# rapidsai/cudf

Hardware: NVIDIA H100
Metric: sort_by_key_rows_per_s (higher is better)
Workload: dtype int64

## Files before the change

cudf_b200/csrc/radix_sort.cu:

```cuda
#include "common.cuh"
#include "device_utils.cuh"

#include <algorithm>
#include <cmath>
#include <cstdlib>
#include <type_traits>

namespace b2 {
namespace {

constexpr int RADIX_BITS = 8;
constexpr int RADIX      = 256;
constexpr uint32_t FLAG_AGG  = 1u << 30;
constexpr uint32_t FLAG_INCL = 2u << 30;
constexpr uint32_t VAL_MASK  = (1u << 30) - 1;

struct pass_plan {
  int32_t trivial;
  int32_t key_src;
  int32_t key_dst;
  int32_t idx_src;
  int32_t idx_dst;
  int32_t last;
  int32_t hybrid;
// ... 784 lines not shown
    }
    if constexpr (RANGE) {
      dstd[j] = (uint8_t)d;
      if (q < tile_n) static_cast<UK*>(s_kdst[d])[dst[j]] = untwiddle_rt<UK>(k, a.kind, desc);
    } else if (write_keys && q < tile_n && (!(MIX || EST) || dst[j] != 0xFFFFFFFFu)) {
      if (!a.pairs && pl.last && !pl.hybrid) k = untwiddle_rt<UK>(k, a.kind, desc);
      kdst[dst[j]] = k;
    }
  }
  if (a.pairs) {
    ranker_barrier(THREADS);
#pragma unroll
    for (int i = 0; i < IPT; ++i) s_vals[pos[i]] = idx[i];
    ranker_barrier(THREADS);
    VT* idst = reinterpret_cast<VT*>(pl.idx_dst == 0 ? a.idx_bufs[0] : (pl.idx_dst == 1 ? a.idx_bufs[1] : a.idx_bufs[2]));
#pragma unroll
    for (int j = 0; j < IPT; ++j) {
      const uint32_t q = j * THREADS + tid;
      if constexpr (RANGE) {
        if (q < tile_n) static_cast<VT*>(s_vdst[dstd[j]])[dst[j]] = s_vals[q];
      } else {
        if (q < tile_n && (!(MIX || EST) || dst[j] != 0xFFFFFFFFu)) idst[dst[j]] = s_vals[q];
      }
    }
  }
}

template <typename UK, bool MIX = false>
__global__ void finalize_kernel(pass_args a, int64_t n, int raw, int pre_idx_buf, int carry_bytes)
{
  if (a.ctl->any_pass != 0) return;
  if (carry_bytes) {
    const int64_t stride = (int64_t)gridDim.x * blockDim.x;
    for (int64_t i = (int64_t)blockIdx.x * blockDim.x + threadIdx.x; i < n; i += stride) {
      if (carry_bytes == 8) reinterpret_cast<uint64_t*>(a.idx_bufs[0])[i] = static_cast<const uint64_t*>(a.val_in)[i];
      else reinterpret_cast<uint32_t*>(a.idx_bufs[0])[i] = static_cast<const uint32_t*>(a.val_in)[i];
      if (a.keep_keys && raw) {
        UK k = static_cast<const UK*>(a.key_bufs[0])[i];
        if constexpr (MIX) k = (UK)mix64((uint64_t)k);
        static_cast<UK*>(const_cast<void*>(a.key_bufs[1]))[i] = k;
      }
    }
    return;
  }
  const int64_t stride = (int64_t)gridDim.x * blockDim.x;
  for (int64_t i = (int64_t)blockIdx.x * blockDim.x + threadIdx.x; i < n; i += stride) {
    if (a.pairs) {
      if (raw) a.idx_bufs[0][i] = (int32_t)i;
      else if (pre_idx_buf != 0) a.idx_bufs[0][i] = a.idx_bufs[1][i];
      if (a.keep_keys && raw) {
        UK k = static_cast<const UK*>(a.key_bufs[0])[i];
        if constexpr (MIX) k = (UK)mix64((uint64_t)k);
        static_cast<UK*>(const_cast<void*>(a.key_bufs[1]))[i] = k;
      }
    } else {
      static_cast<UK*>(const_cast<void*>(a.key_bufs[1]))[i] = static_cast<const UK*>(a.key_bufs[0])[i];
    }
  }
}

constexpr int FIX_THREADS = 256;
constexpr int FIX_IPT     = 8;
constexpr int FIX_TILE    = FIX_THREADS * FIX_IPT;
constexpr int FIX_HALO    = 64;

struct seg_walk {
  int left, before;
  bool all_equal, cut;
};
template <typename UK, int FIX_FAST, typename KeyAt>
__device__ __forceinline__ seg_walk segment_walk(const KeyAt& key_at, UK k, int shift, int lmax, int rmax)
{
  const UK pf = k >> shift;
  seg_walk w{0, 0, true, false};
  bool in_l = true, in_r = true;
#pragma unroll
  for (int s = 1; s <= FIX_FAST; ++s) {
    const UK ol = key_at(-s);
    const UK orr = key_at(s);
    in_l = in_l && s <= lmax && (UK)(ol >> shift) == pf;
    in_r = in_r && s <= rmax && (UK)(orr >> shift) == pf;
    w.left += in_l ? 1 : 0;
    w.before += (in_l && ol <= k) ? 1 : 0;
    w.before += (in_r && orr < k) ? 1 : 0;
    w.all_equal = w.all_equal && (!in_l || ol == k) && (!in_r || orr == k);
  }
  int right = 0;
  if (in_l) {
    for (;;) {
      if (w.left == lmax) { w.cut = lmax == FIX_HALO; break; }
      const UK o = key_at(-w.left - 1);
      if ((UK)(o >> shift) != pf) break;
      ++w.left;
      w.before += o <= k ? 1 : 0;
      w.all_equal = w.all_equal && o == k;
    }
  }
  if (in_r) {
    right = FIX_FAST;
    for (;;) {
      if (right == rmax) { w.cut = w.cut || rmax == FIX_HALO; break; }
      const UK o = key_at(right + 1);
      if ((UK)(o >> shift) != pf) break;
      ++right;
      w.before += o < k ? 1 : 0;
      w.all_equal = w.all_equal && o == k;
    }
  }
  return w;
}

template <typename UK, typename VT, int FIX_FAST>
__global__ void __launch_bounds__(FIX_THREADS) segment_fix_kernel(pass_args a, int64_t n)
{
  if (!a.ctl->hybrid || a.ctl->fix_fast != (FIX_FAST ? 1 : 0)) return;
  __shared__ UK sk[FIX_TILE + 2 * FIX_HALO];
  const int shift = a.ctl->fix_shift;
  const UK* __restrict__ keys = static_cast<const UK*>(a.ctl->fix_key_buf == 1 ? a.key_bufs[1] : a.key_bufs[2]);
  const VT* __restrict__ vin  = reinterpret_cast<const VT*>(a.ctl->fix_idx_buf == 1 ? a.idx_bufs[1] : a.idx_bufs[2]);
  VT* __restrict__ vout = reinterpret_cast<VT*>(a.idx_bufs[0]);
  UK* __restrict__ kout = static_cast<UK*>(const_cast<void*>(a.key_bufs[1]));
  const UK desc = (UK)a.desc_mask;
  const int64_t ntiles = (n + FIX_TILE - 1) / FIX_TILE;
  for (int64_t tile = blockIdx.x; tile < ntiles; tile += gridDim.x) {
    const int64_t base = tile * FIX_TILE;
    __syncthreads();
    for (int q = threadIdx.x; q < FIX_TILE + 2 * FIX_HALO; q += FIX_THREADS) {
      const int64_t g = base - FIX_HALO + q;
      sk[q] = (g >= 0 && g < n) ? ld_stream(keys + g) : UK(0);
    }
    __syncthreads();
#pragma unroll
    for (int j = 0; j < FIX_IPT; ++j) {
      const int i = j * FIX_THREADS + threadIdx.x;
      const int64_t gi = base + i;
      if (gi >= n) continue;
      VT v{};
      if (a.pairs) v = ld_stream(vin + gi);
      const UK k  = sk[FIX_HALO + i];
      const int lmax = (int)(gi < FIX_HALO ? gi : (int64_t)FIX_HALO);
      const int rmax = (int)(n - 1 - gi < FIX_HALO ? n - 1 - gi : (int64_t)FIX_HALO);
      const seg_walk w = segment_walk<UK, FIX_FAST>([&](int o) { return sk[FIX_HALO + i + o]; }, k, shift, lmax, rmax);
      int64_t dst = gi - w.left + w.before;
      if (w.cut) {
        dst = gi;
        if (!w.all_equal) atomicOr(&a.ctl->overflow, 1u);
      }
      if (a.pairs) vout[dst] = v;
      else kout[dst] = untwiddle_rt<UK>(k, a.kind, desc);
    }
  }
}

constexpr int RANGE_THREADS     = 512;
constexpr int RANGE_WARPS       = RANGE_THREADS / 32;
constexpr int RANGE_IPT         = RANGE_CAP / RANGE_THREADS;
constexpr int RANGE_BUCKET_BITS = 13;
constexpr int RANGE_BUCKETS     = 1 << RANGE_BUCKET_BITS;
constexpr int RANGE_BUCKET_CAP  = FIX_HALO;
constexpr int RANGE_SLOTS       = RANGE_BUCKETS + RANGE_BUCKETS / 16;

size_t range_sort_smem(bool est)
{
  return 128 + sizeof(uint64_t) * (RANGE_CAP + 2) +
         (est ? sizeof(uint32_t) * (RANGE_SLOTS + RANGE_CAP) : sizeof(uint32_t) * RANGE_BUCKETS + sizeof(uint16_t) * RANGE_CAP);
}

__global__ void range_bounds_kernel(pass_args a, int64_t n, uint32_t* __restrict__ bounds, int nranges)
{
  const int i = blockIdx.x * blockDim.x + threadIdx.x;
  if (i > nranges) return;
  const uint64_t* __restrict__ keys = static_cast<const uint64_t*>(a.ctl->fix_key_buf == 1 ? a.key_bufs[1] : a.key_bufs[2]);
  const int sh = a.ctl->range_shift;
  const uint64_t mask = (uint64_t)nranges - 1;
  int64_t lo = 0, hi = n;
  while (lo < hi) {
    const int64_t mid = (lo + hi) >> 1;
    if ((int64_t)((keys[mid] >> sh) & mask) < i) lo = mid + 1;
    else hi = mid;
  }
  bounds[i] = (uint32_t)lo;
}

struct range_window {
  int base;
  bool bulk;
};
template <typename T>
__device__ __forceinline__ range_window range_window_load(T* sdst, const T* __restrict__ g, int64_t s, int m, uint32_t mbar)
{
  constexpr int PER = 16 / sizeof(T);
  const int off  = (int)((reinterpret_cast<uintptr_t>(g) & 15) / sizeof(T));
  const bool bulk = (reinterpret_cast<uintptr_t>(g) % sizeof(T)) == 0 && s >= off && m + off >= PER;
  const int bulk_rows = bulk ? (m + off) / PER * PER : 0;
  if (bulk) {
    if constexpr (EMU_BUILD) {
      for (int q = threadIdx.x; q < bulk_rows; q += RANGE_THREADS) sdst[q] = g[q - off];
    } else {
      if (threadIdx.x == 0) bulk_copy_to_smem(sdst, g - off, (uint32_t)(sizeof(T) * bulk_rows), mbar);
    }
    for (int r = bulk_rows - off + (int)threadIdx.x; r < m; r += RANGE_THREADS) sdst[off + r] = g[r];
  } else {
    for (int q = threadIdx.x; q < m; q += RANGE_THREADS) sdst[q] = ld_stream(g + q);
  }
  return {bulk ? off : 0, bulk};
}

__global__ void __launch_bounds__(RADIX) range_est_bounds_kernel(pass_args a, uint32_t cap, uint32_t* __restrict__ est)
{
  __shared__ uint32_t s_lb[RADIX + 1];
  __shared__ uint32_t s_wsum[RADIX / 32];
  constexpr int R = RADIX * RADIX;
  const int d7 = blockIdx.x, d6 = threadIdx.x;
  const uint64_t* __restrict__ keys = static_cast<const uint64_t*>(a.ctl->fix_key_buf == 1 ? a.key_bufs[1] : a.key_bufs[2]);
  auto count = [&](int e) { return min(a.ctl->base[1][7][e] - (uint32_t)e * cap, cap); };
  const uint32_t before = warp_sum(d6 < d7 ? count(d6) : 0u);
  if ((d6 & 31) == 0) s_wsum[d6 >> 5] = before;
  const uint32_t w0 = (uint32_t)d7 * cap, wn = count(d7);
  uint32_t lo = 0, hi = wn;
  while (lo < hi) {
    const uint32_t mid = (lo + hi) >> 1;
    if ((int)((keys[w0 + mid] >> 48) & 255u) < d6) lo = mid + 1;
    else hi = mid;
  }
  s_lb[d6] = lo;
  if (d6 == 0) s_lb[RADIX] = wn;
  __syncthreads();
  uint32_t dense = 0;
  for (int w = 0; w < RADIX / 32; ++w) dense += s_wsum[w];
  const uint32_t end = s_lb[d6 + 1];
  const int i = d7 * RADIX + d6;
  est[i]         = w0 + lo;
  est[R + i]     = end > lo ? end - lo : 0u;
  est[2 * R + i] = dense + lo;
}

#ifdef B2_RANGE_PROBE
constexpr int RANGE_PROBE_CTAS   = 1 << 17;
constexpr int RANGE_PROBE_STAMPS = 8;
__device__ long long g_range_probe[RANGE_PROBE_STAMPS + 2][RANGE_PROBE_CTAS];
void* g_range_probe_ptr()
{
  void* p = nullptr;
  cudaGetSymbolAddress(&p, g_range_probe);
  return p;
}
#define RANGE_PROBE_STAMP(i)                                                                  \
  do {                                                                                        \
    if (threadIdx.x == 0 && blockIdx.x < RANGE_PROBE_CTAS) g_range_probe[i][blockIdx.x] = clock64(); \
  } while (0)
#define RANGE_PROBE_SYNC() __syncthreads()
#else
#define RANGE_PROBE_STAMP(i) do {} while (0)
#define RANGE_PROBE_SYNC() do {} while (0)
#endif

__device__ __attribute__((noinline)) uint32_t range_rank_keys(const uint32_t* s_ord, const uint64_t* sk, uint32_t start, uint32_t end,
                                                              uint32_t r, uint64_t k)
{
  uint32_t before = 0;
  for (uint32_t q = start; q < end; ++q) {
    const uint32_t rq = s_ord[q] & 0xffffu;
    const uint64_t kq = sk[rq];
    before += (kq < k || (kq == k && rq < r)) ? 1u : 0u;
  }
  return before;
}

template <typename VT, bool EST = false>
__global__ void __launch_bounds__(RANGE_THREADS, 1) range_sort_kernel(pass_args a, const uint32_t* __restrict__ bounds)
{
  RANGE_PROBE_STAMP(0);
  using UK = uint64_t;
  B2_DYNAMIC_SMEM(smem_raw);
  uint32_t* s_misc = reinterpret_cast<uint32_t*>(smem_raw);
  UK* s_keys       = reinterpret_cast<UK*>(smem_raw + 128);
  VT* s_vals       = reinterpret_cast<VT*>(s_keys);
  uint32_t* s_cnt  = reinterpret_cast<uint32_t*>(s_keys + RANGE_CAP + 2);
  uint16_t* s_perm = reinterpret_cast<uint16_t*>(s_cnt + (EST ? RANGE_SLOTS : RANGE_BUCKETS));
  uint32_t* s_ord  = reinterpret_cast<uint32_t*>(s_perm);

  const int tid = threadIdx.x, lane = tid & 31, warp = tid >> 5;
  const int64_t s = bounds[blockIdx.x];
  int m;
  int64_t o = s;
  if constexpr (EST) {
    m = (int)bounds[gridDim.x + blockIdx.x];
    o = bounds[2 * gridDim.x + blockIdx.x];
  } else {
    m = (int)(bounds[blockIdx.x + 1] - s);
  }
  if (m == 0) return;
  if (m > RANGE_CAP) {
    if (tid == 0) atomicOr(&a.ctl->overflow, 1u);
    return;
  }
#ifdef B2_RANGE_PROBE
  if (tid == 0 && blockIdx.x < RANGE_PROBE_CTAS) {
    unsigned smid;
    asm volatile("mov.u32 %0, %%smid;" : "=r"(smid));
    g_range_probe[RANGE_PROBE_STAMPS][blockIdx.x]     = smid;
    g_range_probe[RANGE_PROBE_STAMPS + 1][blockIdx.x] = m;
  }
#endif
  const UK* __restrict__ keys = static_cast<const UK*>(a.ctl->fix_key_buf == 1 ? a.key_bufs[1] : a.key_bufs[2]) + s;
  const VT* __restrict__ vin  = reinterpret_cast<const VT*>(a.ctl->fix_idx_buf == 1 ? a.idx_bufs[1] : a.idx_bufs[2]) + s;
  VT* __restrict__ vout = reinterpret_cast<VT*>(a.idx_bufs[0]) + o;
  UK* __restrict__ kout = static_cast<UK*>(const_cast<void*>(a.key_bufs[1])) + o;

  const uint64_t below = a.ctl->vary & ((1ull << a.ctl->range_shift) - 1);
  const uint32_t vhi = (uint32_t)(below >> 32), vlo = (uint32_t)below;
  const int top = vhi ? 64 - __clz((int)vhi) : (vlo ? 32 - __clz((int)vlo) : 0);
  const int want = m > 1 ? 32 - __clz(m - 1) : 0;
  const int nb = min(min(want, RANGE_BUCKET_BITS), top);
  const int bshift = top - nb;
  const uint32_t bmask = (1u << nb) - 1;
  const int lp = max(nb - 9, 0);
  const int per = 1 << lp;
  auto bucket = [&](UK k) { return (uint32_t)(k >> bshift) & bmask; };
  const int dshift = max(bshift - 16, 0);
  auto digest = [&](UK k) { return (uint32_t)(k >> dshift) << 16; };
  const int pad = lp ? lp : 5;
  auto slot = [&](uint32_t b) {
    if constexpr (EST) return b + (b >> pad);
    else return ((b & (uint32_t)(per - 1)) << 9) | (b >> lp);
  };
  auto own = [&](int j) {
    if constexpr (EST) return (int)slot((uint32_t)(tid * per + j));
    else return (j << 9) | tid;
  };

  const uint32_t mbar_k = EMU_BUILD ? 0u : (uint32_t)__cvta_generic_to_shared(s_misc);
  const uint32_t mbar_v = EMU_BUILD ? 0u : (uint32_t)__cvta_generic_to_shared(s_misc + 2);
  if constexpr (!EMU_BUILD) {
    if (tid == 0) {
      mbar_init_one(mbar_k);
      mbar_init_one(mbar_v);
    }
  }
  if (tid == 0) s_misc[4] = 0;
  const int last = EST ? (int)slot(bmask) : (int)bmask;
  for (int i = tid; i <= last; i += RANGE_THREADS) s_cnt[i] = 0;
  __syncthreads();

  const range_window kw = range_window_load(s_keys, keys, s, m, mbar_k);
  if constexpr (!EMU_BUILD) {
    if (tid == 0 && a.pairs) {
      const uintptr_t lo = reinterpret_cast<uintptr_t>(vin) & ~uintptr_t(15);
      const uintptr_t hi = (reinterpret_cast<uintptr_t>(vin + m) + 15) & ~uintptr_t(15);
      asm volatile("cp.async.bulk.prefetch.L2.global [%0], %1;" ::"l"(lo), "r"((uint32_t)(hi - lo)) : "memory");
    }
    if (kw.bulk) mbar_wait_phase0(mbar_k);
  }
  __syncthreads();
  RANGE_PROBE_STAMP(1);
  const UK* sk = s_keys + kw.base;

  for (int r = tid; r < m; r += RANGE_THREADS) atomicAdd(&s_cnt[slot(bucket(sk[r]))], 1u);
  __syncthreads();
  RANGE_PROBE_STAMP(2);
  uint32_t c[1 << (RANGE_BUCKET_BITS - 9)];
  uint32_t tot = 0;
  bool big = false;
#pragma unroll
  for (int j = 0; j < (1 << (RANGE_BUCKET_BITS - 9)); ++j) {
    c[j] = (j < per && tid <= (int)bmask) ? s_cnt[own(j)] : 0u;
    tot += c[j];
    big = big || c[j] > (uint32_t)RANGE_BUCKET_CAP;
  }
  if (big) s_misc[4] = 1;
  const uint32_t inc = warp_inclusive_sum(tot);
  if (lane == 31) s_misc[16 + warp] = inc;
  __syncthreads();
  if (s_misc[4]) {
    if (tid == 0) atomicOr(&a.ctl->overflow, 1u);
    return;
  }
  {
    uint32_t run = inc - tot;
    for (int w = 0; w < warp; ++w) run += s_misc[16 + w];
#pragma unroll
    for (int j = 0; j < (1 << (RANGE_BUCKET_BITS - 9)); ++j) {
      if (j < per && tid <= (int)bmask) s_cnt[own(j)] = run;
      run += c[j];
    }
  }
  __syncthreads();
  RANGE_PROBE_STAMP(3);
  if constexpr (EST) {
    for (int r = tid; r < m; r += RANGE_THREADS) {
      const UK k = sk[r];
      s_ord[atomicAdd(&s_cnt[slot(bucket(k))], 1u)] = digest(k) | (uint32_t)r;
    }
  } else {
    for (int r = tid; r < m; r += RANGE_THREADS) s_perm[atomicAdd(&s_cnt[slot(bucket(sk[r]))], 1u)] = (uint16_t)r;
  }
  __syncthreads();
  RANGE_PROBE_STAMP(4);

  uint32_t pk[RANGE_IPT];
#pragma unroll
  for (int i = 0; i < RANGE_IPT; ++i) {
    const int p = tid + RANGE_THREADS * i;
    if (p >= m) break;
    if constexpr (EST) {
      const uint32_t e = s_ord[p];
      const uint32_t r = e & 0xffffu;
      const UK k = sk[r];
      const uint32_t b = bucket(k);
      const uint32_t end = s_cnt[slot(b)];
      const uint32_t start = b ? s_cnt[slot(b - 1)] : 0u;
      uint32_t before = 0;
      bool tie = false;
      for (uint32_t q = start; q < end; ++q) {
        const uint32_t eq = s_ord[q];
        before += eq < e ? 1u : 0u;
        tie = tie || ((eq ^ e) < 0x10000u && eq != e);
      }
      if (tie) before = range_rank_keys(s_ord, sk, start, end, r, k);
      pk[i] = (start + before) | r << 16;
    } else {
      const uint32_t r = s_perm[p];
      const UK k = sk[r];
      const uint32_t b = bucket(k);
      const uint32_t end = s_cnt[slot(b)];
      const uint32_t start = b ? s_cnt[slot(b - 1)] : 0u;
      uint32_t before = 0;
      for (uint32_t q = start; q < end; ++q) {
        const uint32_t rq = s_perm[q];
        const UK kq = sk[rq];
        before += (kq < k || (kq == k && rq < r)) ? 1u : 0u;
      }
      pk[i] = (start + before) | r << 16;
    }
  }
  __syncthreads();
  RANGE_PROBE_STAMP(5);

  range_window vw{0, false};
  if (a.pairs) vw = range_window_load(s_vals, vin, s, m, mbar_v);
#pragma unroll
  for (int i = 0; i < RANGE_IPT; ++i) {
    if (tid + RANGE_THREADS * i >= m) break;
    s_perm[pk[i] & 0xffffu] = (uint16_t)(pk[i] >> 16);
  }
  if constexpr (!EMU_BUILD) {
    if (vw.bulk) mbar_wait_phase0(mbar_v);
  }
  __syncthreads();
  RANGE_PROBE_STAMP(6);
  if (a.pairs) {
    const VT* sv = s_vals + vw.base;
    for (int r = tid; r < m; r += RANGE_THREADS) vout[r] = sv[s_perm[r]];
  } else {
    const UK desc = (UK)a.desc_mask;
    for (int r = tid; r < m; r += RANGE_THREADS) kout[r] = untwiddle_rt<UK>(sk[s_perm[r]], a.kind, desc);
  }
  RANGE_PROBE_SYNC();
  RANGE_PROBE_STAMP(7);
}

__global__ void reverse_nan_prefix_kernel(int32_t* idx, const uint32_t* nan_count)
{
  const uint32_t m = *nan_count;
  const int64_t stride = (int64_t)gridDim.x * blockDim.x;
  for (int64_t i = (int64_t)blockIdx.x * blockDim.x + threadIdx.x; i < m / 2; i += stride) {
    int32_t x = idx[i], y = idx[m - 1 - i];
    idx[i] = y;
    idx[m - 1 - i] = x;
  }
}

constexpr int CP_THREADS = 256;
constexpr int CP_ROWS    = 2048;

__global__ void __launch_bounds__(CP_THREADS) valid_count_kernel(const uint32_t* __restrict__ mask, int64_t bit_offset,
                                                                  int64_t n, uint32_t* __restrict__ tile_valid)
{
  const int64_t tile = (int64_t)blockIdx.x * (CP_THREADS / 32) + (threadIdx.x >> 5);
  const int64_t ntiles = (n + CP_ROWS - 1) / CP_ROWS;
  if (tile >= ntiles) return;
  const int64_t row0 = tile * CP_ROWS;
  const int64_t last_word = (bit_offset + n - 1) >> 5;
  uint32_t c = 0;
  for (int w = lane_id(); w < CP_ROWS / 32; w += 32) {
    int64_t r = row0 + (int64_t)w * 32;
    if (r < n) {
      uint32_t bits = load_mask_word_unaligned(mask, bit_offset + r, last_word);
      int64_t rem = n - r;
      if (rem < 32) bits &= (1u << rem) - 1u;
      c += __popc(bits);
    }
  }
  c = warp_sum(c);
  if (lane_id() == 0) tile_valid[tile] = c;
}

__global__ void __launch_bounds__(1024) scan_tiles_kernel(uint32_t* __restrict__ tile_valid, int64_t ntiles,
                                                          uint32_t* __restrict__ total)
{
  __shared__ uint32_t wsum[32];
  __shared__ uint32_t carry;
  if (threadIdx.x == 0) carry = 0;
  __syncthreads();
  for (int64_t b = 0; b < ntiles; b += 1024) {
    int64_t i = b + threadIdx.x;
    uint32_t v = i < ntiles ? tile_valid[i] : 0;
    uint32_t inc = warp_inclusive_sum(v);
    if (lane_id() == 31) wsum[threadIdx.x >> 5] = inc;
    __syncthreads();
    uint32_t woff = 0;
    for (int w = 0; w < (int)(threadIdx.x >> 5); ++w) woff += wsum[w];
    uint32_t c = carry;
    if (i < ntiles) tile_valid[i] = c + woff + inc - v;
    __syncthreads();
    if (threadIdx.x == 1023) carry = c + woff + inc;
    __syncthreads();
  }
  if (threadIdx.x == 0) *total = carry;
}

template <typename UK>
__global__ void __launch_bounds__(CP_THREADS) compact_kernel(const UK* __restrict__ keys, const uint32_t* __restrict__ mask,
                                                             int64_t bit_offset, int64_t n, int kind, UK desc_mask,
                                                             const uint32_t* __restrict__ tile_valid_excl,
                                                             UK* __restrict__ out_keys, int32_t* __restrict__ out_valid_idx,
                                                             int32_t* __restrict__ out_null_idx)
{
  __shared__ uint32_t wcount[CP_ROWS / 32];
  const int64_t tile = blockIdx.x;
  const int64_t row0 = tile * CP_ROWS;
  const int64_t last_word = (bit_offset + n - 1) >> 5;
  const uint32_t vbase = tile_valid_excl[tile];
  const uint32_t nbase = (uint32_t)row0 - vbase;
  uint32_t bits = 0;
  if (threadIdx.x < CP_ROWS / 32) {
    int64_t r = row0 + (int64_t)threadIdx.x * 32;
    if (r < n) {
      bits = load_mask_word_unaligned(mask, bit_offset + r, last_word);
      int64_t rem = n - r;
      if (rem < 32) bits &= (1u << rem) - 1u;
    }
    wcount[threadIdx.x] = __popc(bits);
  }
  __syncthreads();
  for (int w = threadIdx.x >> 5; w < CP_ROWS / 32; w += CP_THREADS / 32) {
    int64_t r = row0 + (int64_t)w * 32 + lane_id();
    uint32_t before = 0;
    for (int j = lane_id(); j < w; j += 32) before += wcount[j];
    before = warp_sum(before);
    bool in = r < n;
    bool valid = false;
    if (in) {
      uint32_t wb = load_mask_word_unaligned(mask, bit_offset + row0 + (int64_t)w * 32, last_word);
      valid = (wb >> lane_id()) & 1u;
    }
    unsigned vb = __ballot_sync(0xffffffffu, valid);
    unsigned nb = __ballot_sync(0xffffffffu, in && !valid);
    if (valid) {
      uint32_t o = vbase + before + __popc(vb & lanemask_lt());
      out_keys[o]      = twiddle_rt<UK>(keys[r], kind, desc_mask);
      out_valid_idx[o] = (int32_t)r;
    } else if (in) {
      uint32_t o = nbase + ((uint32_t)w * 32 - before) + __popc(nb & lanemask_lt());
      out_null_idx[o] = (int32_t)r;
    }
  }
}

int64_t portion_rows(int tile)
{
  static const int64_t lim = [] {
    const char* e = std::getenv("B2_SORT_PORTION");
    int64_t v = e ? std::atoll(e) : 0;
    if (v <= 0) v = (int64_t(1) << 30) - 16384;
    return v;
  }();
  return std::max<int64_t>(tile, lim / tile * tile);
}

template <typename UK, typename Shape, typename VT, bool CARRY, bool MIX, bool RANGE = false, bool EST = false>
struct onesweep_passes {
  static constexpr int TILE = Shape::tile;
  static constexpr size_t SMEM = (sizeof(UK) > sizeof(VT) ? sizeof(UK) : sizeof(VT)) * (size_t)TILE +
                                 sizeof(uint32_t) * (2 * (Shape::threads / 32) * RADIX + 3 * RADIX + 16) +
                                 (RANGE ? (sizeof(UK) + 2 * sizeof(void*)) * RADIX + (size_t)TILE : 0);
  static constexpr size_t CTL_BYTES = (sizeof(sort_ctl) + 255) / 256 * 256;
  const int64_t n, plim, nportions;
  const size_t hist_bytes, cnt_bytes, head_bytes, status_per;
  dbuf work;

  onesweep_passes(int64_t rows, int passes, size_t hist, size_t tail_bytes, cudaStream_t stream, int extra_tiles = 0)
    : n(rows), plim(portion_rows(TILE)), nportions((n + plim - 1) / plim), hist_bytes(hist),
      cnt_bytes((sizeof(uint32_t) * passes * nportions + 255) / 256 * 256), head_bytes(CTL_BYTES + hist_bytes + cnt_bytes + tail_bytes),
      status_per(sizeof(uint32_t) * RADIX * (size_t)((std::min(n, plim) + TILE - 1) / TILE + extra_tiles)),
      work(head_bytes + status_per * passes * nportions, stream)
  {
    static std::atomic<uint64_t> attr_done{0};
    once_per_device(attr_done, [] {
      B2_CUDA_TRY(cudaFuncSetAttribute(onesweep_kernel<UK, Shape, VT, CARRY, MIX, RANGE, EST>, cudaFuncAttributeMaxDynamicSharedMemorySize,
                                       (int)SMEM));
    });
  }
  sort_ctl* ctl() const { return work.as<sort_ctl>(); }
  uint32_t* hist() const { return reinterpret_cast<uint32_t*>(work.as<char>() + CTL_BYTES); }
  void* tail() const { return work.as<char>() + CTL_BYTES + hist_bytes + cnt_bytes; }
  void zero_head(cudaStream_t stream) const { B2_CUDA_TRY(cudaMemsetAsync(work.ptr, 0, head_bytes, stream)); }

  void run(pass_args& a, int slot, const char* scope, cudaStream_t stream, int extra_tiles = 0) const
  {
    for (int64_t q = 0; q < nportions; ++q) {
      const int64_t start = q * plim;
      const int64_t pn = std::min(plim, n - start);
      const int64_t ntiles = (pn + TILE - 1) / TILE + extra_tiles;
      a.portion_start = start;
      a.portion_n = (uint32_t)pn;
      a.portion_parity = (int)(q & 1);
      a.has_next_portion = q + 1 < nportions;
      a.status = reinterpret_cast<uint32_t*>(work.as<char>() + head_bytes + (size_t)(slot * nportions + q) * status_per);
      a.tile_counter = reinterpret_cast<uint32_t*>(work.as<char>() + CTL_BYTES + hist_bytes) + slot * nportions + q;
      B2_CUDA_TRY(cudaMemsetAsync(a.status, 0, sizeof(uint32_t) * RADIX * (size_t)ntiles, stream));
      prof_scope ps(scope, stream);
      B2_LAUNCH((onesweep_kernel<UK, Shape, VT, CARRY, MIX, RANGE, EST>), (unsigned)ntiles, Shape::threads + 32 * LBW, SMEM, stream, a);
    }
  }
};

constexpr int64_t RANGE_MIN_ROWS = int64_t(1) << 27;
int range_env()
{
  static int v = [] {
    const char* e = std::getenv("B2_SORT_RANGE");
    return e ? (std::atoi(e) != 0 ? 1 : 0) : -1;
  }();
  return v;
}

int64_t hybrid_min_rows()
{
  static int64_t v = [] {
    const char* off = std::getenv("B2_SORT_HYBRID");
    if (off && std::atoi(off) == 0) return INT64_MAX;
    const char* e = std::getenv("B2_SORT_HYBRID_MIN");
    return e ? (int64_t)std::atoll(e) : (int64_t(1) << 16);
  }();
  return v;
}

__global__ void range_est_plan_kernel(sort_ctl* ctl, uint32_t cap)
{
  const int d = threadIdx.x;
  ctl->base[0][6][d] = (uint32_t)d * cap;
  ctl->base[0][7][d] = (uint32_t)d * cap;
  if (d < 8) {
    pass_plan pl{};
    pl.trivial = d < 6;
    if (d >= 6) {
      pl.key_src = d == 6 ? 0 : 1;
      pl.key_dst = d == 6 ? 1 : 2;
      pl.idx_src = d == 6 ? -1 : 2;
      pl.idx_dst = d == 6 ? 2 : 1;
      pl.last    = d == 7;
      pl.hybrid  = 1;
    }
    ctl->plan[d] = pl;
  }
  if (d == 0) {
    ctl->any_pass    = 2;
    ctl->hybrid      = 1;
    ctl->range       = 1;
    ctl->range_shift = 48;
    ctl->range_bits  = 16;
    ctl->fix_shift   = 48;
    ctl->fix_key_buf = 2;
    ctl->fix_idx_buf = 1;
    ctl->overflow    = 0;
  }
}

__global__ void range_est_tiles_kernel(const sort_ctl* ctl, uint32_t cap, int tile, uint2* __restrict__ tiles)
{
  __shared__ uint32_t s_wsum[RADIX / 32];
  const int d = threadIdx.x;
  const uint32_t cnt = min(ctl->base[1][6][d] - (uint32_t)d * cap, cap);
  const uint32_t nt = (cnt + (uint32_t)tile - 1) / (uint32_t)tile;
  const uint32_t inc = warp_inclusive_sum(nt);
  if ((d & 31) == 31) s_wsum[d >> 5] = inc;
  __syncthreads();
  uint32_t first = inc - nt, total = 0;
  for (int w = 0; w < RADIX / 32; ++w) {
    first += w < (d >> 5) ? s_wsum[w] : 0u;
    total += s_wsum[w];
  }
  for (uint32_t k = 0; k < nt; ++k) {
    const uint32_t off = k * (uint32_t)tile;
    const uint32_t t = first + k;
    tiles[t] = make_uint2((uint32_t)d * cap + off, min((uint32_t)tile, cnt - off) | (t + 1 == total ? 0x80000000u : 0u));
  }
}

template <typename UK, typename Shape, typename VT, bool CARRY>
bool run_est_range(const UK* raw_keys, UK* keys_out, UK* k1, UK* k2, int32_t* idx_out, int32_t* v1, int32_t* v2, int64_t n, uint32_t cap,
                   int kind, UK desc_mask, bool pairs, const void* val_in, cudaStream_t stream)
{
  static_assert(sizeof(UK) == 8, "the estimated-base range tier sorts 64-bit keys");
  constexpr int TILE = Shape::tile;
  const int64_t ntiles = (n + TILE - 1) / TILE + RADIX;
  const size_t table_bytes = (sizeof(uint2) * ntiles + 255) / 256 * 256;
  const onesweep_passes<UK, Shape, VT, CARRY, false, false, true> passes(n, 2, 0, table_bytes, stream, RADIX);
  {
    static std::atomic<uint64_t> attr_done{0};
    once_per_device(attr_done, [] {
      B2_CUDA_TRY(cudaFuncSetAttribute(range_sort_kernel<VT, true>, cudaFuncAttributeMaxDynamicSharedMemorySize, (int)range_sort_smem(true)));
    });
  }
  sort_ctl* const ctl = passes.ctl();
  uint2* const tiles = static_cast<uint2*>(passes.tail());
  passes.zero_head(stream);
  B2_LAUNCH(range_est_plan_kernel, 1, RADIX, 0, stream, ctl, cap);
  pass_args a{};
  a.key_bufs[0] = raw_keys;
  a.key_bufs[1] = k1;
  a.key_bufs[2] = k2;
  a.idx_bufs[0] = idx_out;
  a.idx_bufs[1] = v2;
  a.idx_bufs[2] = v1;
  a.ctl = ctl;
  a.kind = kind;
  a.pairs = pairs ? 1 : 0;
  a.val_in = val_in;
  a.desc_mask = (uint64_t)desc_mask;
  a.est_cap = cap;
  a.pass = 6;
  passes.run(a, 0, "onesweep", stream);
  B2_LAUNCH(range_est_tiles_kernel, 1, RADIX, 0, stream, (const sort_ctl*)ctl, cap, TILE, tiles);
  a.pass = 7;
  a.est_tiles = tiles;
  passes.run(a, 1, "onesweep", stream, RADIX);
  a.key_bufs[1] = keys_out;
  dbuf bounds(sizeof(uint32_t) * 3 * RADIX * RADIX, stream);
  {
    prof_scope ps("range_bounds", stream);
    B2_LAUNCH(range_est_bounds_kernel, RADIX, RADIX, 0, stream, a, cap, bounds.as<uint32_t>());
  }
  {
    prof_scope ps("segment_fix", stream);
    B2_LAUNCH((range_sort_kernel<VT, true>), RADIX * RADIX, RANGE_THREADS, range_sort_smem(true), stream, a, bounds.as<const uint32_t>());
  }
  uint32_t overflow = 0;
  B2_CUDA_TRY(cudaMemcpyAsync(&overflow, &ctl->overflow, sizeof(overflow), cudaMemcpyDeviceToHost, stream));
  B2_CUDA_TRY(cudaStreamSynchronize(stream));
  return overflow == 0;
}

template <typename UK, typename Shape, typename VT = uint32_t, bool CARRY = false, bool MIX = false>
void run_radix_cfg(const UK* raw_keys, UK* bufA, UK* bufB, int32_t* idx_out, int32_t* idx_tmp, int32_t* idx_tmp2, int pre_idx_buf, int64_t n,
                   int kind, bool descending, bool pairs, cudaStream_t stream, int first_pass = 0, int last_pass = 7,
                   bool keep_keys = false, const void* val_in = nullptr, uint32_t* top_digit_base_out = nullptr, uint32_t est_cap = 0,
                   void* est_buf = nullptr)
{
  constexpr int NP = sizeof(UK);
  const bool raw = raw_keys != nullptr;
  const UK desc_mask = descending ? ~UK(0) : UK(0);

  if constexpr (sizeof(UK) == 8 && !MIX) {
    if (est_cap != 0 && raw && first_pass == 0 && last_pass >= NP - 1 && !keep_keys) {
      const bool done =
        pairs ? run_est_range<UK, Shape, VT, CARRY>(raw_keys, bufA, bufA, bufB, idx_out, static_cast<int32_t*>(est_buf), idx_tmp, n, est_cap,
                                                    kind, desc_mask, true, val_in, stream)
              : run_est_range<UK, Shape, VT, CARRY>(raw_keys, bufA, static_cast<UK*>(est_buf), bufB, nullptr, nullptr, nullptr, n, est_cap,
                                                    kind, desc_mask, false, val_in, stream);
      if (done) return;
    }
  }

  const onesweep_passes<UK, Shape, VT, CARRY, MIX> passes(n, NP, sizeof(uint32_t) * NP * RADIX, 0, stream);
  sort_ctl* const ctl = passes.ctl();
  uint32_t* const ghist = passes.hist();
  if constexpr (sizeof(UK) == 8 && !MIX) {
    static std::atomic<uint64_t> attr_done{0};
    once_per_device(attr_done, [] {
      B2_CUDA_TRY(cudaFuncSetAttribute(range_sort_kernel<VT>, cudaFuncAttributeMaxDynamicSharedMemorySize, (int)range_sort_smem(false)));
    });
  }

  bool try_hybrid = sizeof(UK) == 8 && !MIX && raw && first_pass == 0 && last_pass >= NP - 1 && !keep_keys && n >= hybrid_min_rows();
  const int force_range = range_env();
  bool try_range = try_hybrid && force_range != 0 && (force_range == 1 || n >= RANGE_MIN_ROWS);

  for (;;) {
    passes.zero_head(stream);
    {
      int grid = (int)std::min<int64_t>((n + 512 * 16 - 1) / (512 * 16), num_sms() * 4);
      grid = std::max(grid, 1);
      const UK* hkeys = raw ? raw_keys : bufA;
      uint32_t* nanp = (raw && kind == (int)key_kind::FLOAT) ? &ctl->nan_count : nullptr;
      const uint32_t span_mask = ((last_pass >= NP - 1 ? (1u << NP) : (1u << (last_pass + 1))) - 1u) & ~((1u << std::max(first_pass, 0)) - 1u);
      if (try_hybrid) {
        {
          prof_scope ps("histogram", stream);
          B2_LAUNCH((histogram_kernel<UK, MIX>), grid, 512, 0, stream, hkeys, n, raw ? 1 : 0, kind, desc_mask, ghist, nanp, 0xf0u,
                    (const int32_t*)nullptr, &ctl->vary);
        }
        B2_LAUNCH(plan_kernel, 1, RADIX, 0, stream, ghist, NP, (uint32_t)n, raw ? 1 : 0, pre_idx_buf, ctl, first_pass, last_pass, 1, 1,
                  try_range ? 1 : 0);
        {
          prof_scope ps("histogram", stream);
          B2_LAUNCH((histogram_kernel<UK, MIX>), grid, 512, 0, stream, hkeys, n, raw ? 1 : 0, kind, desc_mask, ghist, (uint32_t*)nullptr, 0x0fu,
                    &ctl->need_low, (unsigned long long*)nullptr);
        }
        B2_LAUNCH(plan_kernel, 1, RADIX, 0, stream, ghist, NP, (uint32_t)n, raw ? 1 : 0, pre_idx_buf, ctl, first_pass, last_pass, 1, 2,
                  try_range ? 1 : 0);
      } else {
        {
          prof_scope ps("histogram", stream);
          B2_LAUNCH((histogram_kernel<UK, MIX>), grid, 512, 0, stream, hkeys, n, raw ? 1 : 0, kind, desc_mask, ghist, nanp, span_mask,
                    (const int32_t*)nullptr, (unsigned long long*)nullptr);
        }
        B2_LAUNCH(plan_kernel, 1, RADIX, 0, stream, ghist, NP, (uint32_t)n, raw ? 1 : 0, pre_idx_buf, ctl, first_pass, last_pass, 0, 0);
      }
    }

    {
      static const int force_fix = [] {
        const char* e = std::getenv("B2_SORT_FIX_FAST");
        return e ? (std::atoi(e) != 0 ? 1 : 0) : -1;
      }();
      if (force_fix >= 0 && try_hybrid) B2_LAUNCH(set_fix_fast_kernel, 1, 1, 0, stream, ctl, force_fix);
    }
    pass_args a{};
    a.key_bufs[0] = raw_keys;
    a.key_bufs[1] = bufA;
    a.key_bufs[2] = bufB;
    a.idx_bufs[0] = idx_out;
    a.idx_bufs[1] = idx_tmp;
    a.idx_bufs[2] = idx_tmp2;
    a.ctl = ctl;
    a.kind = kind;
    a.pairs = pairs ? 1 : 0;
    a.keep_keys = keep_keys ? 1 : 0;
    a.val_in = val_in;
    a.desc_mask = (uint64_t)desc_mask;
    uint32_t skip_mask = 0;
    bool plan_hybrid = true;
    int range_bits = 0;
    static const int64_t readback_min = [] {
      const char* e = std::getenv("B2_SORT_PLAN_READBACK_MIN");
      return e ? (int64_t)std::atoll(e) : (int64_t(1) << 22);
    }();
    if (n >= readback_min || try_range) {
      pass_plan hp[8];
      int32_t hflag = 0, hrange[3] = {0, 0, 0};
      B2_CUDA_TRY(cudaMemcpyAsync(hp, &ctl->plan[0], sizeof(pass_plan) * 8, cudaMemcpyDeviceToHost, stream));
      B2_CUDA_TRY(cudaMemcpyAsync(&hflag, &ctl->hybrid, sizeof(int32_t), cudaMemcpyDeviceToHost, stream));
      if (try_range) B2_CUDA_TRY(cudaMemcpyAsync(hrange, &ctl->range, sizeof(hrange), cudaMemcpyDeviceToHost, stream));
      B2_CUDA_TRY(cudaStreamSynchronize(stream));
      for (int p = 0; p < NP; ++p)
        if (hp[p].trivial) skip_mask |= 1u << p;
      plan_hybrid = hflag != 0;
      range_bits = hrange[0] ? hrange[2] : 0;
    }
    for (int p = std::max(0, first_pass); p < NP && p <= last_pass; ++p) {
      if ((skip_mask >> p) & 1u) continue;
      a.pass = p;
      passes.run(a, p, "onesweep", stream);
    }
    if constexpr (sizeof(UK) == 8 && !MIX) {
      if (try_hybrid && plan_hybrid && range_bits) {
        const int nranges = 1 << range_bits;
        dbuf bounds(sizeof(uint32_t) * (nranges + 1), stream);
        {
          prof_scope ps("range_bounds", stream);
          B2_LAUNCH(range_bounds_kernel, (nranges + 256) / 256, 256, 0, stream, a, n, bounds.as<uint32_t>(), nranges);
        }
        prof_scope ps("segment_fix", stream);
        B2_LAUNCH((range_sort_kernel<VT>), nranges, RANGE_THREADS, range_sort_smem(false), stream, a, bounds.as<const uint32_t>());
      } else if (try_hybrid && plan_hybrid) {
        const int64_t ntiles = (n + FIX_TILE - 1) / FIX_TILE;
        const int grid = (int)std::min<int64_t>(ntiles, num_sms() * 8);
        prof_scope ps("segment_fix", stream);
        B2_LAUNCH((segment_fix_kernel<UK, VT, 0>), grid, FIX_THREADS, 0, stream, a, n);
        B2_LAUNCH((segment_fix_kernel<UK, VT, 3>), grid, FIX_THREADS, 0, stream, a, n);
      }
    }
    {
      int grid = (int)std::min<int64_t>((n + 255) / 256, num_sms() * 8);
      B2_LAUNCH((finalize_kernel<UK, MIX>), std::max(grid, 1), 256, 0, stream, a, n, raw ? 1 : 0, pre_idx_buf, CARRY ? (int)sizeof(VT) : 0);
    }
    if (!try_hybrid || !plan_hybrid) break;
    uint32_t overflow = 0;
    B2_CUDA_TRY(cudaMemcpyAsync(&overflow, &ctl->overflow, sizeof(overflow), cudaMemcpyDeviceToHost, stream));
    B2_CUDA_TRY(cudaStreamSynchronize(stream));
    if (!overflow) break;
    if (range_bits) {
      try_range = false;
      continue;
    }
    try_hybrid = false;
  }
  if (pairs && raw && kind == (int)key_kind::FLOAT && descending) {
// ... 600 lines not shown
```

Baseline: 25.59 billion.

## Rank range-sort buckets with warp ballots over start flags and bounded window

In the estimated-range sort path, bucket starts are marked with a flag bit in the ordered array. Warp ballots then find each element's bucket bounds without reading the count array, and small buckets are ranked by digest comparison over a fixed window of eight. Large buckets or digest ties fall back to a key-compare routine that rescans for the bounds, and two elements per thread are processed at once. Each element scatters directly into a separate sorted array that reuses the count storage, and the value-window load is issued earlier so it overlaps with ranking. This aims to remove the unbounded per-element scan and the extra pass through registers, at the cost of more fallback work when buckets exceed the window.

After: 26.29 billion, median of 6. 1.03x the previous value.

```diff
diff --git a/cudf_b200/csrc/radix_sort.cu b/cudf_b200/csrc/radix_sort.cu
--- a/cudf_b200/csrc/radix_sort.cu
+++ b/cudf_b200/csrc/radix_sort.cu
@@ -1063,16 +1063,24 @@
 #define RANGE_PROBE_SYNC() do {} while (0)
 #endif
 
-__device__ __attribute__((noinline)) uint32_t range_rank_keys(const uint32_t* s_ord, const uint64_t* sk, uint32_t start, uint32_t end,
-                                                              uint32_t r, uint64_t k)
-{
+constexpr uint32_t RANGE_START  = 0x8000u;
+constexpr uint32_t RANGE_ROW    = RANGE_CAP - 1;
+constexpr int      RANGE_WINDOW = 8;
+
+__device__ __attribute__((noinline)) uint32_t range_rank_keys(const uint32_t* s_ord, const uint64_t* keys, int p, int m)
+{
+  int start = p, end = p + 1;
+  while (!(s_ord[start] & RANGE_START)) --start;
+  while (end < m && !(s_ord[end] & RANGE_START)) ++end;
+  const uint32_t r = s_ord[p] & RANGE_ROW;
+  const uint64_t k = keys[r];
   uint32_t before = 0;
-  for (uint32_t q = start; q < end; ++q) {
-    const uint32_t rq = s_ord[q] & 0xffffu;
-    const uint64_t kq = sk[rq];
+  for (int q = start; q < end; ++q) {
+    const uint32_t rq = s_ord[q] & RANGE_ROW;
+    const uint64_t kq = keys[rq];
     before += (kq < k || (kq == k && rq < r)) ? 1u : 0u;
   }
-  return before;
+  return (uint32_t)start + before;
 }
 
 template <typename VT, bool EST = false>
@@ -1086,7 +1094,8 @@
   VT* s_vals       = reinterpret_cast<VT*>(s_keys);
   uint32_t* s_cnt  = reinterpret_cast<uint32_t*>(s_keys + RANGE_CAP + 2);
   uint16_t* s_perm = reinterpret_cast<uint16_t*>(s_cnt + (EST ? RANGE_SLOTS : RANGE_BUCKETS));
-  uint32_t* s_ord  = reinterpret_cast<uint32_t*>(s_perm);
+  uint32_t* s_ord    = reinterpret_cast<uint32_t*>(s_perm);
+  uint16_t* s_sorted = EST ? reinterpret_cast<uint16_t*>(s_cnt) : s_perm;
 
   const int tid = threadIdx.x, lane = tid & 31, warp = tid >> 5;
   const int64_t s = bounds[blockIdx.x];
@@ -1184,9 +1193,10 @@
     if (tid == 0) atomicOr(&a.ctl->overflow, 1u);
     return;
   }
+  uint32_t first = inc - tot;
+  for (int w = 0; w < warp; ++w) first += s_misc[16 + w];
   {
-    uint32_t run = inc - tot;
-    for (int w = 0; w < warp; ++w) run += s_misc[16 + w];
+    uint32_t run = first;
 #pragma unroll
     for (int j = 0; j < (1 << (RANGE_BUCKET_BITS - 9)); ++j) {
       if (j < per && tid <= (int)bmask) s_cnt[own(j)] = run;
@@ -1206,28 +1216,60 @@
   __syncthreads();
   RANGE_PROBE_STAMP(4);
 
+  range_window vw{0, false};
   uint32_t pk[RANGE_IPT];
-#pragma unroll
-  for (int i = 0; i < RANGE_IPT; ++i) {
-    const int p = tid + RANGE_THREADS * i;
-    if (p >= m) break;
-    if constexpr (EST) {
-      const uint32_t e = s_ord[p];
-      const uint32_t r = e & 0xffffu;
-      const UK k = sk[r];
-      const uint32_t b = bucket(k);
-      const uint32_t end = s_cnt[slot(b)];
-      const uint32_t start = b ? s_cnt[slot(b - 1)] : 0u;
-      uint32_t before = 0;
-      bool tie = false;
-      for (uint32_t q = start; q < end; ++q) {
-        const uint32_t eq = s_ord[q];
-        before += eq < e ? 1u : 0u;
-        tie = tie || ((eq ^ e) < 0x10000u && eq != e);
-      }
-      if (tie) before = range_rank_keys(s_ord, sk, start, end, r, k);
-      pk[i] = (start + before) | r << 16;
-    } else {
+  if constexpr (EST) {
+    if (a.pairs) vw = range_window_load(s_vals, vin, s, m, mbar_v);
+    uint32_t q = first;
+#pragma unroll
+    for (int j = 0; j < (1 << (RANGE_BUCKET_BITS - 9)); ++j) {
+      if (c[j]) s_ord[q] |= RANGE_START;
+      q += c[j];
+    }
+    __syncthreads();
+    auto rank = [&](int p, uint32_t& e) {
+      e = p < m ? s_ord[p] : RANGE_START;
+      const uint32_t fb = __ballot_sync(~0u, p < 32 || (s_ord[p - 32] & RANGE_START));
+      const uint32_t fc = __ballot_sync(~0u, e & RANGE_START);
+      const uint32_t fa = __ballot_sync(~0u, p + 32 >= m || (s_ord[p + 32] & RANGE_START));
+      const int P = p - lane;
+      const uint32_t upto = (2u << lane) - 1u;
+      const uint32_t sb = fc & upto, sa = fc & ~upto;
+      const int st = sb ? P + 31 - __clz((int)sb) : P - 1 - __clz((int)(fb | 1u));
+      const int en = sa ? P - 1 + __ffs((int)sa) : P + 31 + __ffs((int)(fa | 0x80000000u));
+      const int len = en - st <= RANGE_WINDOW && p < m ? en - st : 0;
+      const uint32_t de = e >> 16;
+      uint32_t lt = 0, le = 0;
+#pragma unroll
+      for (int j = 0; j < RANGE_WINDOW; ++j) {
+        if (j < len) {
+          const uint32_t d = s_ord[st + j] >> 16;
+          lt += (d - de) >> 31;
+          le += (d - de - 1) >> 31;
+        }
+      }
+      return le == lt + 1 ? (uint32_t)st + lt : ~0u;
+    };
+    for (int p = tid; p - lane < m; p += 2 * RANGE_THREADS) {
+      uint32_t e[2], dst[2];
+#pragma unroll
+      for (int u = 0; u < 2; ++u) dst[u] = rank(p + u * RANGE_THREADS, e[u]);
+#pragma unroll
+      for (int u = 0; u < 2; ++u) {
+        const int pu = p + u * RANGE_THREADS;
+        if (pu < m) {
+          if (dst[u] == ~0u) dst[u] = range_rank_keys(s_ord, keys, pu, m);
+          s_sorted[dst[u]] = (uint16_t)(e[u] & RANGE_ROW);
+        }
+      }
+    }
+    __syncthreads();
+    RANGE_PROBE_STAMP(5);
+  } else {
+#pragma unroll
+    for (int i = 0; i < RANGE_IPT; ++i) {
+      const int p = tid + RANGE_THREADS * i;
+      if (p >= m) break;
       const uint32_t r = s_perm[p];
       const UK k = sk[r];
       const uint32_t b = bucket(k);
@@ -1241,16 +1283,15 @@
       }
       pk[i] = (start + before) | r << 16;
     }
-  }
-  __syncthreads();
-  RANGE_PROBE_STAMP(5);
-
-  range_window vw{0, false};
-  if (a.pairs) vw = range_window_load(s_vals, vin, s, m, mbar_v);
-#pragma unroll
-  for (int i = 0; i < RANGE_IPT; ++i) {
-    if (tid + RANGE_THREADS * i >= m) break;
-    s_perm[pk[i] & 0xffffu] = (uint16_t)(pk[i] >> 16);
+    __syncthreads();
+    RANGE_PROBE_STAMP(5);
+
+    if (a.pairs) vw = range_window_load(s_vals, vin, s, m, mbar_v);
+#pragma unroll
+    for (int i = 0; i < RANGE_IPT; ++i) {
+      if (tid + RANGE_THREADS * i >= m) break;
+      s_perm[pk[i] & 0xffffu] = (uint16_t)(pk[i] >> 16);
+    }
   }
   if constexpr (!EMU_BUILD) {
     if (vw.bulk) mbar_wait_phase0(mbar_v);
@@ -1259,10 +1300,10 @@
   RANGE_PROBE_STAMP(6);
   if (a.pairs) {
     const VT* sv = s_vals + vw.base;
-    for (int r = tid; r < m; r += RANGE_THREADS) vout[r] = sv[s_perm[r]];
+    for (int r = tid; r < m; r += RANGE_THREADS) vout[r] = sv[s_sorted[r]];
   } else {
     const UK desc = (UK)a.desc_mask;
-    for (int r = tid; r < m; r += RANGE_THREADS) kout[r] = untwiddle_rt<UK>(sk[s_perm[r]], a.kind, desc);
+    for (int r = tid; r < m; r += RANGE_THREADS) kout[r] = untwiddle_rt<UK>(sk[s_sorted[r]], a.kind, desc);
   }
   RANGE_PROBE_SYNC();
   RANGE_PROBE_STAMP(7);
```

## Widen estimated range-sort blocks and batch bucket rank walks per thread

Applied to the files above, without the earlier changes.

The estimated-bounds range sort kernel now runs 1024 threads per block instead of 512, and its digest packing shrinks to 15 row bits to fit. The per-row rank walk is restructured to process four rows together with branch-free less-than and less-or-equal counts over a shared maximum length, falling back to a full key compare only on digest ties. Slot padding is also simplified to a fixed shift. The aim is more memory-level parallelism and fewer divergent loops in the segment-fix stage, at the cost of redundant clamped loads when bucket lengths differ and higher register pressure.

After: 25.43 billion before, 26.35 billion after, median of 6. +3.6%, better.

```diff
diff --git a/cudf_b200/csrc/radix_sort.cu b/cudf_b200/csrc/radix_sort.cu
--- a/cudf_b200/csrc/radix_sort.cu
+++ b/cudf_b200/csrc/radix_sort.cu
@@ -960,17 +960,21 @@
   }
 }
 
-constexpr int RANGE_THREADS     = 512;
-constexpr int RANGE_WARPS       = RANGE_THREADS / 32;
-constexpr int RANGE_IPT         = RANGE_CAP / RANGE_THREADS;
+template <bool EST>
+constexpr int range_log_threads = EST && !EMU_BUILD ? 10 : 9;
+constexpr int RANGE_THREADS     = 1 << range_log_threads<false>;
 constexpr int RANGE_BUCKET_BITS = 13;
 constexpr int RANGE_BUCKETS     = 1 << RANGE_BUCKET_BITS;
 constexpr int RANGE_BUCKET_CAP  = FIX_HALO;
-constexpr int RANGE_SLOTS       = RANGE_BUCKETS + RANGE_BUCKETS / 16;
+constexpr int RANGE_SLOTS       = RANGE_BUCKETS + RANGE_BUCKETS / 32;
+constexpr int RANGE_WALK_ROWS   = 4;
+constexpr uint32_t RANGE_ROW_MASK = (1u << 15) - 1;
+
+constexpr int range_head_bytes(bool est) { return est ? 256 : 128; }
 
 size_t range_sort_smem(bool est)
 {
-  return 128 + sizeof(uint64_t) * (RANGE_CAP + 2) +
+  return range_head_bytes(est) + sizeof(uint64_t) * (RANGE_CAP + 2) +
          (est ? sizeof(uint32_t) * (RANGE_SLOTS + RANGE_CAP) : sizeof(uint32_t) * RANGE_BUCKETS + sizeof(uint16_t) * RANGE_CAP);
 }
 
@@ -994,7 +998,7 @@
   int base;
   bool bulk;
 };
-template <typename T>
+template <int THREADS, typename T>
 __device__ __forceinline__ range_window range_window_load(T* sdst, const T* __restrict__ g, int64_t s, int m, uint32_t mbar)
 {
   constexpr int PER = 16 / sizeof(T);
@@ -1003,13 +1007,13 @@
   const int bulk_rows = bulk ? (m + off) / PER * PER : 0;
   if (bulk) {
     if constexpr (EMU_BUILD) {
-      for (int q = threadIdx.x; q < bulk_rows; q += RANGE_THREADS) sdst[q] = g[q - off];
+      for (int q = threadIdx.x; q < bulk_rows; q += THREADS) sdst[q] = g[q - off];
     } else {
       if (threadIdx.x == 0) bulk_copy_to_smem(sdst, g - off, (uint32_t)(sizeof(T) * bulk_rows), mbar);
     }
-    for (int r = bulk_rows - off + (int)threadIdx.x; r < m; r += RANGE_THREADS) sdst[off + r] = g[r];
+    for (int r = bulk_rows - off + (int)threadIdx.x; r < m; r += THREADS) sdst[off + r] = g[r];
   } else {
-    for (int q = threadIdx.x; q < m; q += RANGE_THREADS) sdst[q] = ld_stream(g + q);
+    for (int q = threadIdx.x; q < m; q += THREADS) sdst[q] = ld_stream(g + q);
   }
   return {bulk ? off : 0, bulk};
 }
@@ -1068,7 +1072,7 @@
 {
   uint32_t before = 0;
   for (uint32_t q = start; q < end; ++q) {
-    const uint32_t rq = s_ord[q] & 0xffffu;
+    const uint32_t rq = s_ord[q] & RANGE_ROW_MASK;
     const uint64_t kq = sk[rq];
     before += (kq < k || (kq == k && rq < r)) ? 1u : 0u;
   }
@@ -1076,13 +1080,16 @@
 }
 
 template <typename VT, bool EST = false>
-__global__ void __launch_bounds__(RANGE_THREADS, 1) range_sort_kernel(pass_args a, const uint32_t* __restrict__ bounds)
+__global__ void __launch_bounds__(1 << range_log_threads<EST>, 1) range_sort_kernel(pass_args a, const uint32_t* __restrict__ bounds)
 {
   RANGE_PROBE_STAMP(0);
   using UK = uint64_t;
+  constexpr int LT  = range_log_threads<EST>;
+  constexpr int RT  = 1 << LT;
+  constexpr int IPT = RANGE_CAP / RT;
   B2_DYNAMIC_SMEM(smem_raw);
   uint32_t* s_misc = reinterpret_cast<uint32_t*>(smem_raw);
-  UK* s_keys       = reinterpret_cast<UK*>(smem_raw + 128);
+  UK* s_keys       = reinterpret_cast<UK*>(smem_raw + range_head_bytes(EST));
   VT* s_vals       = reinterpret_cast<VT*>(s_keys);
   uint32_t* s_cnt  = reinterpret_cast<uint32_t*>(s_keys + RANGE_CAP + 2);
   uint16_t* s_perm = reinterpret_cast<uint16_t*>(s_cnt + (EST ? RANGE_SLOTS : RANGE_BUCKETS));
@@ -1123,19 +1130,18 @@
   const int nb = min(min(want, RANGE_BUCKET_BITS), top);
   const int bshift = top - nb;
   const uint32_t bmask = (1u << nb) - 1;
-  const int lp = max(nb - 9, 0);
+  const int lp = max(nb - LT, 0);
   const int per = 1 << lp;
   auto bucket = [&](UK k) { return (uint32_t)(k >> bshift) & bmask; };
   const int dshift = max(bshift - 16, 0);
-  auto digest = [&](UK k) { return (uint32_t)(k >> dshift) << 16; };
-  const int pad = lp ? lp : 5;
+  auto digest = [&](UK k) { return (uint32_t)(k >> dshift) << 15; };
   auto slot = [&](uint32_t b) {
-    if constexpr (EST) return b + (b >> pad);
-    else return ((b & (uint32_t)(per - 1)) << 9) | (b >> lp);
+    if constexpr (EST) return b + (b >> 5);
+    else return ((b & (uint32_t)(per - 1)) << LT) | (b >> lp);
   };
   auto own = [&](int j) {
     if constexpr (EST) return (int)slot((uint32_t)(tid * per + j));
-    else return (j << 9) | tid;
+    else return (j << LT) | tid;
   };
 
   const uint32_t mbar_k = EMU_BUILD ? 0u : (uint32_t)__cvta_generic_to_shared(s_misc);
@@ -1148,10 +1154,10 @@
   }
   if (tid == 0) s_misc[4] = 0;
   const int last = EST ? (int)slot(bmask) : (int)bmask;
-  for (int i = tid; i <= last; i += RANGE_THREADS) s_cnt[i] = 0;
+  for (int i = tid; i <= last; i += RT) s_cnt[i] = 0;
   __syncthreads();
 
-  const range_window kw = range_window_load(s_keys, keys, s, m, mbar_k);
+  const range_window kw = range_window_load<RT>(s_keys, keys, s, m, mbar_k);
   if constexpr (!EMU_BUILD) {
     if (tid == 0 && a.pairs) {
       const uintptr_t lo = reinterpret_cast<uintptr_t>(vin) & ~uintptr_t(15);
@@ -1164,14 +1170,14 @@
   RANGE_PROBE_STAMP(1);
   const UK* sk = s_keys + kw.base;
 
-  for (int r = tid; r < m; r += RANGE_THREADS) atomicAdd(&s_cnt[slot(bucket(sk[r]))], 1u);
+  for (int r = tid; r < m; r += RT) atomicAdd(&s_cnt[slot(bucket(sk[r]))], 1u);
   __syncthreads();
   RANGE_PROBE_STAMP(2);
-  uint32_t c[1 << (RANGE_BUCKET_BITS - 9)];
+  uint32_t c[1 << (RANGE_BUCKET_BITS - LT)];
   uint32_t tot = 0;
   bool big = false;
 #pragma unroll
-  for (int j = 0; j < (1 << (RANGE_BUCKET_BITS - 9)); ++j) {
+  for (int j = 0; j < (1 << (RANGE_BUCKET_BITS - LT)); ++j) {
     c[j] = (j < per && tid <= (int)bmask) ? s_cnt[own(j)] : 0u;
     tot += c[j];
     big = big || c[j] > (uint32_t)RANGE_BUCKET_CAP;
@@ -1188,7 +1194,7 @@
     uint32_t run = inc - tot;
     for (int w = 0; w < warp; ++w) run += s_misc[16 + w];
 #pragma unroll
-    for (int j = 0; j < (1 << (RANGE_BUCKET_BITS - 9)); ++j) {
+    for (int j = 0; j < (1 << (RANGE_BUCKET_BITS - LT)); ++j) {
       if (j < per && tid <= (int)bmask) s_cnt[own(j)] = run;
       run += c[j];
     }
@@ -1196,38 +1202,60 @@
   __syncthreads();
   RANGE_PROBE_STAMP(3);
   if constexpr (EST) {
-    for (int r = tid; r < m; r += RANGE_THREADS) {
+    for (int r = tid; r < m; r += RT) {
       const UK k = sk[r];
       s_ord[atomicAdd(&s_cnt[slot(bucket(k))], 1u)] = digest(k) | (uint32_t)r;
     }
   } else {
-    for (int r = tid; r < m; r += RANGE_THREADS) s_perm[atomicAdd(&s_cnt[slot(bucket(sk[r]))], 1u)] = (uint16_t)r;
+    for (int r = tid; r < m; r += RT) s_perm[atomicAdd(&s_cnt[slot(bucket(sk[r]))], 1u)] = (uint16_t)r;
   }
   __syncthreads();
   RANGE_PROBE_STAMP(4);
 
-  uint32_t pk[RANGE_IPT];
-#pragma unroll
-  for (int i = 0; i < RANGE_IPT; ++i) {
-    const int p = tid + RANGE_THREADS * i;
-    if (p >= m) break;
-    if constexpr (EST) {
-      const uint32_t e = s_ord[p];
-      const uint32_t r = e & 0xffffu;
-      const UK k = sk[r];
-      const uint32_t b = bucket(k);
-      const uint32_t end = s_cnt[slot(b)];
-      const uint32_t start = b ? s_cnt[slot(b - 1)] : 0u;
-      uint32_t before = 0;
-      bool tie = false;
-      for (uint32_t q = start; q < end; ++q) {
-        const uint32_t eq = s_ord[q];
-        before += eq < e ? 1u : 0u;
-        tie = tie || ((eq ^ e) < 0x10000u && eq != e);
-      }
-      if (tie) before = range_rank_keys(s_ord, sk, start, end, r, k);
-      pk[i] = (start + before) | r << 16;
-    } else {
+  uint32_t pk[IPT];
+  if constexpr (EST) {
+#pragma unroll
+    for (int i0 = 0; i0 < IPT; i0 += RANGE_WALK_ROWS) {
+      if (tid + RT * i0 >= m) break;
+      uint32_t e[RANGE_WALK_ROWS], start[RANGE_WALK_ROWS], end[RANGE_WALK_ROWS];
+#pragma unroll
+      for (int g = 0; g < RANGE_WALK_ROWS; ++g) e[g] = tid + RT * (i0 + g) < m ? s_ord[tid + RT * (i0 + g)] : 0u;
+      uint32_t len = 0;
+#pragma unroll
+      for (int g = 0; g < RANGE_WALK_ROWS; ++g) {
+        const bool in = tid + RT * (i0 + g) < m;
+        const uint32_t b = bucket(sk[e[g] & RANGE_ROW_MASK]);
+        end[g] = in ? s_cnt[slot(b)] : 1u;
+        start[g] = in && b ? s_cnt[slot(b - 1)] : 0u;
+        len = max(len, end[g] - start[g]);
+      }
+      auto lo = [&](int g) { return e[g] & ~RANGE_ROW_MASK; };
+      auto hi = [&](int g) { return (e[g] & ~RANGE_ROW_MASK) + RANGE_ROW_MASK + 1; };
+      uint32_t lt[RANGE_WALK_ROWS] = {}, le[RANGE_WALK_ROWS] = {};
+      for (uint32_t q = 0; q < len; ++q) {
+#pragma unroll
+        for (int g = 0; g < RANGE_WALK_ROWS; ++g) {
+          const uint32_t eq = s_ord[min(start[g] + q, end[g] - 1)];
+          lt[g] += (eq - lo(g)) >> 31;
+          le[g] += (eq - hi(g)) >> 31;
+        }
+      }
+#pragma unroll
+      for (int g = 0; g < RANGE_WALK_ROWS; ++g) {
+        const uint32_t extra = len - (end[g] - start[g]);
+        const uint32_t eq = s_ord[end[g] - 1];
+        lt[g] -= extra * ((eq - lo(g)) >> 31);
+        le[g] -= extra * ((eq - hi(g)) >> 31);
+        const uint32_t r = e[g] & RANGE_ROW_MASK;
+        if (le[g] - lt[g] > 1u) lt[g] = range_rank_keys(s_ord, sk, start[g], end[g], r, sk[r]);
+        pk[i0 + g] = (start[g] + lt[g]) | r << 16;
+      }
+    }
+  } else {
+#pragma unroll
+    for (int i = 0; i < IPT; ++i) {
+      const int p = tid + RT * i;
+      if (p >= m) break;
       const uint32_t r = s_perm[p];
       const UK k = sk[r];
       const uint32_t b = bucket(k);
@@ -1246,10 +1274,10 @@
   RANGE_PROBE_STAMP(5);
 
   range_window vw{0, false};
-  if (a.pairs) vw = range_window_load(s_vals, vin, s, m, mbar_v);
-#pragma unroll
-  for (int i = 0; i < RANGE_IPT; ++i) {
-    if (tid + RANGE_THREADS * i >= m) break;
+  if (a.pairs) vw = range_window_load<RT>(s_vals, vin, s, m, mbar_v);
+#pragma unroll
+  for (int i = 0; i < IPT; ++i) {
+    if (tid + RT * i >= m) break;
     s_perm[pk[i] & 0xffffu] = (uint16_t)(pk[i] >> 16);
   }
   if constexpr (!EMU_BUILD) {
@@ -1259,10 +1287,10 @@
   RANGE_PROBE_STAMP(6);
   if (a.pairs) {
     const VT* sv = s_vals + vw.base;
-    for (int r = tid; r < m; r += RANGE_THREADS) vout[r] = sv[s_perm[r]];
+    for (int r = tid; r < m; r += RT) vout[r] = sv[s_perm[r]];
   } else {
     const UK desc = (UK)a.desc_mask;
-    for (int r = tid; r < m; r += RANGE_THREADS) kout[r] = untwiddle_rt<UK>(sk[s_perm[r]], a.kind, desc);
+    for (int r = tid; r < m; r += RT) kout[r] = untwiddle_rt<UK>(sk[s_perm[r]], a.kind, desc);
   }
   RANGE_PROBE_SYNC();
   RANGE_PROBE_STAMP(7);
@@ -1553,7 +1581,7 @@
   }
   {
     prof_scope ps("segment_fix", stream);
-    B2_LAUNCH((range_sort_kernel<VT, true>), RADIX * RADIX, RANGE_THREADS, range_sort_smem(true), stream, a, bounds.as<const uint32_t>());
+    B2_LAUNCH((range_sort_kernel<VT, true>), RADIX * RADIX, 1 << range_log_threads<true>, range_sort_smem(true), stream, a, bounds.as<const uint32_t>());
   }
   uint32_t overflow = 0;
   B2_CUDA_TRY(cudaMemcpyAsync(&overflow, &ctl->overflow, sizeof(overflow), cudaMemcpyDeviceToHost, stream));
```
